# danieleschmidt/grid-fed-rl-gym

Measured on NVIDIA B200. Metric: env-steps/sec, higher is better.
Workload: dtype f64

## Files before the change

### grid-fed-rl-gym_b200/csrc/gfr_device.cuh

```cuda
#pragma once
#include <math.h>
#include <stdint.h>

#if defined(__CUDACC__)
#define GFR_HD __host__ __device__ __forceinline__
#else
#define GFR_HD inline
#endif

namespace gfr {

enum { SOLVER_SWEEP = 0, SOLVER_NEWTON = 1, SOLVER_SWEEP_TIES = 2 };
enum { BUS_SLACK = 0, BUS_PV = 1, BUS_PQ = 2 };
enum { GEN_SOLAR = 0, GEN_WIND = 1 };
enum { F_E = 0, F_F = 1, F_SCRATCH = 2 };
enum { S_JR = 2, S_P = 4 };
enum { SCRATCH_FIELDS_SWEEP = 2 };
enum { FL_PQ = 1, FL_FROM_IS_PARENT = 2, FL_FIXED_VM = 4, FL_THETA = 8,
       FL_SLACK_PATH = 16,
       FL_C_REG = 32,
       FL_P_REG = 64,
       FL_VALID = 128,
       FL_POOL_SHIFT = 8, FL_POOL_MASK = 0xFFF,
       FL_XSLOT_SHIFT = 20,
       REC_LIST_MASK = 0xFFFFF, REC_KIDX_SHIFT = 20 };
enum { R_TIME = 0, R_FREQ, R_WIND, R_TEMP, R_CLOUD, R_TOTAL_LOSSES, R_EPISODE_REWARD, R_SEED,
       R_DRAWS, R_COUNTS, R_BAT };

struct alignas(16) D2 { double x, y; };
struct alignas(16) I4 { int x, y, z, w; };
GFR_HD int pool_slot_of(int w) { return (w >> FL_POOL_SHIFT) & FL_POOL_MASK; }
GFR_HD int rec_bus(const I4& t) { return (int)((unsigned)t.x & 0xFFFFu); }
GFR_HD int rec_parent(const I4& t) { return (int)((unsigned)t.x >> 16); }
GFR_HD int rec_list(const I4& t) { return t.y & REC_LIST_MASK; }
GFR_HD int rec_kids_x_slot(const I4& t) { return (int)((unsigned)t.y >> REC_KIDX_SHIFT); }
GFR_HD int x_slot_of(int z) { return (int)((unsigned)z >> FL_XSLOT_SHIFT); }
GFR_HD int rec_pool_kids(const I4& t) { return (int)((unsigned)t.w & 0xFFFFu); }
GFR_HD int rec_all_kids(const I4& t) { return (int)((unsigned)t.w >> 16); }

struct Layout {
  int n, nl, L, G, Bt, A, D, m, n_src, R, img_bytes, n_noise, n_pool, k_slack;
  int nrows, P;
  int n_tie;
  int o_tie_ends, o_tie_ptr, o_tie_inc, o_tie_y, o_tie_z, o_tie_rating, o_tie_zinv;
  int o_sched, o_rank, o_rankp, o_branch_of_line, o_inj_ptr, o_inj_idx, o_gen_type;
  int o_gb, o_rating, o_vm_set;
  int o_child_ent, o_child_slot, o_gbd, o_f0;
  int o_kids;
  int o_topo, o_child_idx, o_rx;
  int o_rowrec, sw_rows;
  int o_load_base, o_gen_cap, o_gen_p0, o_gen_p1, o_gen_p2, o_bat_cap, o_bat_rating, o_bat_eff, o_profile;
  double s_base, inv_s_base, load_p_sum;
};

struct EnvCfg {
  double dt, v_min, v_max, f_min, f_max, penalty, load_noise, tol, accel;
  int episode_length, stochastic_loads, weather_variation, max_it;
};

struct SolveStat {
  double max_mismatch;
  int iterations;
  int converged;
};

GFR_HD uint64_t scratch_policy() {
#if defined(__CUDA_ARCH__) && !defined(GFR_NO_L2_POLICY)
  uint64_t pol;
  asm volatile("createpolicy.fractional.L2::evict_last.b64 %0, 1.0;" : "=l"(pol));
  return pol;
#else
  return 0;
#endif
}
GFR_HD D2 ld_scratch(const D2* p, uint64_t pol) {
#if defined(__CUDA_ARCH__) && !defined(GFR_NO_L2_POLICY)
  D2 r;
  asm volatile("ld.global.L1::no_allocate.L2::cache_hint.v2.f64 {%0, %1}, [%2], %3;" : "=d"(r.x), "=d"(r.y) : "l"(p), "l"(pol) : "memory");
  return r;
#elif defined(__CUDA_ARCH__)
  D2 r;
  asm volatile("ld.global.L1::no_allocate.v2.f64 {%0, %1}, [%2];" : "=d"(r.x), "=d"(r.y) : "l"(p) : "memory");
  return r;
#else
  (void)pol;
  return *p;
#endif
}
GFR_HD void st_scratch(D2* p, const D2 v, uint64_t pol) {
#if defined(__CUDA_ARCH__) && !defined(GFR_NO_L2_POLICY)
  asm volatile("st.global.L2::cache_hint.v2.f64 [%0], {%1, %2}, %3;" ::"l"(p), "d"(v.x), "d"(v.y), "l"(pol) : "memory");
// ... 353 lines not shown
template <class G, int LANES>
GFR_HD void flat_start_t(const G& g, const Lanes<LANES>&, const Layout& lay, const int* simg,
                         const double* dimg) {
  const I4* sched = reinterpret_cast<const I4*>(simg + lay.o_sched);
  if (wide_group<LANES>()) {
    for (int p0 = g.lane; p0 < lay.P; p0 += 4 * LANES) {
      I4 t[4]; double vs[4];
#pragma unroll
      for (int u = 0; u < 4; ++u) {
        const int p = p0 + u * LANES;
        t[u].x = t[u].y = t[u].z = t[u].w = 0; vs[u] = 1.0;
        if (p < lay.P) { t[u] = sched[p]; vs[u] = dimg[lay.o_vm_set + p]; }
      }
#pragma unroll
      for (int u = 0; u < 4; ++u) {
        if (!(t[u].z & FL_VALID)) continue;
        D2 v;
        v.x = (t[u].z & FL_FIXED_VM) ? vs[u] : 1.0;
        v.y = 0.0;
        g.ef(rec_bus(t[u])) = v;
      }
    }
  } else
  for (int p = g.lane; p < lay.P; p += LANES) {
    const I4 t = sched[p];
    if (!(t.z & FL_VALID)) continue;
    D2 v;
    v.x = (t.z & FL_FIXED_VM) ? dimg[lay.o_vm_set + p] : 1.0;
    v.y = 0.0;
    g.ef(rec_bus(t)) = v;
  }
  g.sync();
}
template <class G>
GFR_HD void flat_start(const G& g, const Layout& lay, const int* simg, const double* dimg) {
  flat_start_t(g, g, lay, simg, dimg);
}

#ifdef GFR_EMU_STATS
static long long gfr_emu_stats[4];
#endif
struct BranchT { double ga, al, gl, ll; };
GFR_HD BranchT branch_terms(const D2 vk, const D2 vp, const D2 y) {
  const double a = fma(vk.x, vp.x, vk.y * vp.y), s = fma(vk.y, vp.x, -vk.x * vp.y);
  BranchT t;
  t.ga = fma(-y.x, a, -y.y * s); t.al = fma(-y.x, s, y.y * a);
  t.gl = fma(-y.x, a, y.y * s);  t.ll = fma(y.x, s, y.y * a);
  return t;
}

GFR_HD unsigned shr16_pair(unsigned lo, unsigned hi) { return (lo >> 16) | (hi << 16); }
#define GFR_POOL_GATHER(t_, kq_, ...)                                                                              \
  do {                                                                                                             \
    const int npk_ = rec_pool_kids(t_);                                                                            \
    if (wide_group<LANES>() && npk_ <= 8) {                                                                       \
      unsigned w0_ = (unsigned)(kq_).x, w1_ = (unsigned)(kq_).y, w2_ = (unsigned)(kq_).z, w3_ = (unsigned)(kq_).w; \
      _Pragma("unroll 1")                                                                                          \
      for (int j_ = 0; j_ < npk_; ++j_) {                                                                          \
        const int slot = (int)(w0_ & 0xffffu);                                                                     \
        w0_ = shr16_pair(w0_, w1_); w1_ = shr16_pair(w1_, w2_); w2_ = shr16_pair(w2_, w3_); w3_ >>= 16;            \
        __VA_ARGS__                                                                                                \
      }                                                                                                            \
    } else {                                                                                                       \
      const int q1_ = rec_list(t_) + rec_all_kids(t_);                                                             \
      _Pragma("unroll 1")                                                                                          \
      for (int q_ = q1_ - npk_; q_ < q1_; ++q_) {                                                                  \
        const int slot = child_slot[q_];                                                                           \
        __VA_ARGS__                                                                                                \
      }                                                                                                            \
    }                                                                                                              \
  } while (0)

#define GFR_ROW_PIPE_DECL                                                                                          \
  I4 t_next, kq_next; D2 y_next, yd_next, vk_next, vp_next;                                                        \
  t_next.x = t_next.y = t_next.z = t_next.w = 0;                                                                   \
  kq_next = t_next;                                                                                                \
  y_next.x = y_next.y = yd_next.x = yd_next.y = vk_next.x = vk_next.y = vp_next.x = vp_next.y = 0.0
#define GFR_ROW_PIPE_LOAD(pos_)                                                                                    \
  do {                                                                                                             \
    t_next = sched[(pos_)]; y_next = gb[(pos_)]; yd_next = gbd[(pos_)];                                            \
    if (wide_group<LANES>()) kq_next = kids[(pos_)];                                                              \
    if (GFR_PIPE_EF) { vk_next = g.ef(rec_bus(t_next)); vp_next = g.ef(rec_parent(t_next)); }                      \
  } while (0)
#define GFR_ROW_PIPE_FIRST(pos_)                                                                                   \
  do { if (pipe_rows<LANES>()) GFR_ROW_PIPE_LOAD(pos_); } while (0)
#define GFR_ROW_PIPE_TAKE(p_, more_, next_)                                                                        \
  I4 t, kq; D2 yb, yd, vk, vp;                                                                                     \
  kq.x = kq.y = kq.z = kq.w = 0;                                                                                   \
  if (pipe_rows<LANES>()) {                                                                                        \
    t = t_next; yb = y_next; yd = yd_next; kq = kq_next;                                                           \
    if (GFR_PIPE_EF) { vk = vk_next; vp = vp_next; } else { vk = g.ef(rec_bus(t)); vp = g.ef(rec_parent(t)); }     \
    if (more_) GFR_ROW_PIPE_LOAD(next_);                                                                           \
  } else {                                                                                                         \
    t = sched[(p_)]; yb = gb[(p_)]; yd = gbd[(p_)]; vk = g.ef(rec_bus(t)); vp = g.ef(rec_parent(t));               \
    if (wide_group<LANES>()) kq = kids[(p_)];                                                                     \
  }

template <int LANES>
GFR_HD double newton_mismatch(const NGrp<LANES>& g, const Layout& lay, const int* simg, const double* dimg) {
  const int nrows = lay.nrows, np = lay.n_pool;
  const I4* sched = reinterpret_cast<const I4*>(simg + lay.o_sched);
  const int* child_slot = simg + lay.o_child_slot;
  const D2* gb = reinterpret_cast<const D2*>(dimg + lay.o_gb);
  const D2* gbd = reinterpret_cast<const D2*>(dimg + lay.o_gbd);
  const I4* kids = reinterpret_cast<const I4*>(simg + (wide_group<LANES>() ? lay.o_kids : 0));
  double mm = 0.0;
  D2 hf; hf.x = hf.y = 0.0;
  double ps_next = g.pspec((nrows - 1) * LANES + g.lane);
  GFR_ROW_PIPE_DECL;
  GFR_ROW_PIPE_FIRST((nrows - 1) * LANES + g.lane);
  for (int row = nrows - 1; row >= 0; --row) {
    const int p = row * LANES + g.lane;
    GFR_ROW_PIPE_TAKE(p, row > 0, p - LANES);
    const double ps = ps_next;
    if (row > 0) ps_next = g.pspec(p - LANES);
    if (t.z & FL_VALID) {
      const double v2 = fma(vk.x, vk.x, vk.y * vk.y);
      const BranchT bt = branch_terms(vk, vp, yb);
      if (!(t.z & FL_C_REG)) { hf.x = hf.y = 0.0; }
      GFR_POOL_GATHER(t, kq, {
        const D2 fl = g.poolp[3 * np + slot];
        hf.x += fl.x; hf.y += fl.y;
      });
      const double P = fma(yd.x, v2, bt.ga) + hf.x, Q = fma(-yd.y, v2, bt.al) + hf.y;
      double aP = fabs(ps - P), aQ = fabs(Q);
      if ((t.z & (FL_PQ | FL_THETA)) != (FL_PQ | FL_THETA)) {
        if (!(t.z & FL_THETA)) aP = 0.0;
        if (!(t.z & FL_PQ)) aQ = 0.0;
      }
      const double loc = (aQ > aP || aQ != aQ) ? aQ : aP;
      mm = (loc > mm || loc != loc) ? loc : mm;
      hf.x = bt.gl; hf.y = bt.ll;
      if (!(t.z & FL_P_REG)) g.poolp[3 * np + pool_slot_of(t.z)] = hf;
    }
    g.sync();
  }
  return g.gmax_nan(mm);
}

template <int LANES>
GFR_HD void newton_back_update(const NGrp<LANES>& g, const Layout& lay, const int* simg, const D2* f0,
                               double accel) {
  const int nrows = lay.nrows, P = lay.P;
  const I4* sched = reinterpret_cast<const I4*>(simg + lay.o_sched);
  D2 a0, a1, av, b0, b1, bv;
  a0.x = a0.y = a1.x = a1.y = b0.x = b0.y = b1.x = b1.y = bv.x = bv.y = 0.0;
#define GFR_LOAD_MV(row_, m0_, m1_, v_)                                    \
  do {                                                                     \
    const int ps_ = (row_) * LANES + g.lane;                               \
    if (!f0) { m0_ = ld_scratch(g.mg + ps_, g.pol); m1_ = ld_scratch(g.mg + P + ps_, g.pol); } \
    v_ = ld_scratch(g.mg + 2 * P + ps_, g.pol);                                   \
  } while (0)
  D2 hx; hx.x = hx.y = 0.0;
#define GFR_BU_ROW(row_, m0_, m1_, v_)                                     \
  do {                                                                     \
    const int p = (row_) * LANES + g.lane;                                 \
    I4 t;                                                                  \
    D2 e_now;                                                              \
    if (pipe_rows<LANES>()) {                                              \
      t = t_next; e_now = e_next;                                          \
      if ((row_) + 1 < nrows) { t_next = sched[p + LANES]; if (GFR_PIPE_EF) e_next = g.efp[rec_bus(t_next)]; } \
      if (!GFR_PIPE_EF) e_now = g.efp[rec_bus(t)];                         \
    } else { t = sched[p]; e_now = g.efp[rec_bus(t)]; }                    \
    D2 m0 = m0_, m1 = m1_, v = v_;                                         \
    if (f0) {                                                              \
      if (LANES > 32) {                                                    \
        m0 = f0m0_next; m1 = f0m1_next;                                    \
        if ((row_) + 1 < nrows) { f0m0_next = f0[2 * P + p + LANES]; f0m1_next = f0[3 * P + p + LANES]; } \
      } else { m0 = f0[2 * P + p]; m1 = f0[3 * P + p]; }                   \
    }                                                                      \
    if ((row_) + 2 < nrows) GFR_LOAD_MV((row_) + 2, m0_, m1_, v_);         \
    if (t.z & FL_VALID) {                                                  \
      D2 x = hx;                                                           \
      if (!(t.z & FL_P_REG)) x = g.poolp[x_slot_of(t.z)];                  \
      v.x = fma(-m0.x, x.x, fma(-m0.y, x.y, v.x));                         \
      v.y = fma(-m1.x, x.x, fma(-m1.y, x.y, v.y));                         \
      if (rec_pool_kids(t)) g.poolp[rec_kids_x_slot(t)] = v;               \
      hx = v;                                                              \
      double sn, cs;                                                       \
      sincos_small(accel * v.x, &sn, &cs);                                 \
      const double sc = fma(accel, v.y, 1.0);                              \
      D2* const ep = g.efp + rec_bus(t);                                   \
      const D2 e = e_now;                                                  \
      D2 w;                                                                \
      w.x = sc * fma(e.x, cs, -e.y * sn);                                  \
      w.y = sc * fma(e.x, sn, e.y * cs);                                   \
      *ep = w;                                                             \
    }                                                                      \
    g.sync();                                                              \
  } while (0)
  GFR_LOAD_MV(0, a0, a1, av);
  if (nrows > 1) GFR_LOAD_MV(1, b0, b1, bv);
  I4 t_next;
  t_next.x = t_next.y = t_next.z = t_next.w = 0;
  D2 f0m0_next, f0m1_next;
  f0m0_next.x = f0m0_next.y = f0m1_next.x = f0m1_next.y = 0.0;
  D2 e_next; e_next.x = e_next.y = 0.0;
  if (pipe_rows<LANES>()) { t_next = sched[g.lane]; if (GFR_PIPE_EF) e_next = g.efp[rec_bus(t_next)]; }
  if (LANES > 32 && f0) { f0m0_next = f0[2 * P + g.lane]; f0m1_next = f0[3 * P + g.lane]; }
  for (int row = 0; row < nrows; row += 2) {
    GFR_BU_ROW(row, a0, a1, av);
    if (row + 1 < nrows) GFR_BU_ROW(row + 1, b0, b1, bv);
  }
#undef GFR_BU_ROW
#undef GFR_LOAD_MV
}

template <int LANES>
GFR_HD void newton_solve(const NGrp<LANES>& g, const Layout& lay, const int* simg,
                         const double* dimg, double tol, int max_it, double accel,
                         SolveStat* out) {
  const int nrows = lay.nrows, np = lay.n_pool, P = lay.P;
  const I4* sched = reinterpret_cast<const I4*>(simg + lay.o_sched);
  const int* child_slot = simg + lay.o_child_slot;
  const D2* gb = reinterpret_cast<const D2*>(dimg + lay.o_gb);
  const D2* gbd = reinterpret_cast<const D2*>(dimg + lay.o_gbd);
  const D2* f0 = lay.o_f0 >= 0 ? reinterpret_cast<const D2*>(dimg + lay.o_f0) : nullptr;
  const I4* kids = reinterpret_cast<const I4*>(simg + (wide_group<LANES>() ? lay.o_kids : 0));

  out->converged = 0;
  out->iterations = max_it;
  out->max_mismatch = INFINITY;
  double mm_prev = INFINITY, rate = 1.0;

  for (int it = 0; it < max_it; ++it) {
    double mm;
    if (it == 0 && f0 != nullptr) {
      mm = 0.0;
      for (int p = g.lane; p < P; p += LANES) {
        const int fl = sched[p].z;
// ... 4 lines not shown
        const double loc = (aQ > aP || aQ != aQ) ? aQ : aP;
        if (fl & FL_VALID) mm = (loc > mm || loc != loc) ? loc : mm;
      }
      mm = g.gmax_nan(mm);
      out->max_mismatch = mm;
      if (mm < tol) {
        out->converged = 1;
        out->iterations = it + 1;
        break;
      }
      D2 hc; hc.x = hc.y = 0.0;
      double ps_next = g.pspec((nrows - 1) * LANES + g.lane);
      I4 t_next, kq_next; D2 pc_next, i0_next, i1_next, lp_next;
      t_next.x = t_next.y = t_next.z = t_next.w = 0;
      kq_next = t_next;
      pc_next.x = pc_next.y = i0_next.x = i0_next.y = i1_next.x = i1_next.y = lp_next.x = lp_next.y = 0.0;
      if (pipe_rows<LANES>()) {
        const int p0 = (nrows - 1) * LANES + g.lane;
        t_next = sched[p0]; pc_next = f0[5 * P + p0]; i0_next = f0[p0]; i1_next = f0[P + p0]; lp_next = f0[4 * P + p0];
        if (wide_group<LANES>()) kq_next = kids[p0];
      }
      for (int row = nrows - 1; row >= 0; --row) {
        const int p = row * LANES + g.lane;
        I4 t, kq; D2 pc, i0, i1, lp;
        kq.x = kq.y = kq.z = kq.w = 0;
        if (pipe_rows<LANES>()) {
          t = t_next; pc = pc_next; i0 = i0_next; i1 = i1_next; lp = lp_next; kq = kq_next;
          if (row > 0) {
            if (wide_group<LANES>()) kq_next = kids[p - LANES];
            t_next = sched[p - LANES]; pc_next = f0[5 * P + p - LANES];
            i0_next = f0[p - LANES]; i1_next = f0[P + p - LANES]; lp_next = f0[4 * P + p - LANES];
          }
        } else {
          t = sched[p]; pc = f0[5 * P + p]; i0 = f0[p]; i1 = f0[P + p]; lp = f0[4 * P + p];
          if (wide_group<LANES>()) kq = kids[p];
        }
        const double ps = ps_next;
        if (row > 0) ps_next = g.pspec(p - LANES);
        if (t.z & FL_VALID) {
          if (!(t.z & FL_C_REG)) { hc.x = hc.y = 0.0; }
          GFR_POOL_GATHER(t, kq, {
            const D2 cc = g.poolp[2 * np + slot];
            hc.x += cc.x; hc.y += cc.y;
          });
          const D2 sc = hc;
          double r0 = ps - pc.x - sc.x, r1 = 0.0 - pc.y - sc.y;
          if (!(t.z & FL_THETA)) r0 = 0.0;
          if (!(t.z & FL_PQ)) r1 = 0.0;
          D2 v;
          v.x = fma(i0.x, r0, i0.y * r1);
          v.y = fma(i1.x, r0, i1.y * r1);
          hc.x = fma(lp.x, v.x, lp.y * v.y);
          hc.y = fma(-lp.y, v.x, lp.x * v.y);
          st_scratch(g.mg + 2 * P + p, v, g.pol);
          if (!(t.z & FL_P_REG)) g.poolp[2 * np + pool_slot_of(t.z)] = hc;
        }
        g.sync();
      }
      newton_back_update(g, lay, simg, f0, accel);
    } else {
      if (rate * mm_prev * mm_prev < 0.25 * tol) {
#ifdef GFR_EMU_STATS
        ++gfr_emu_stats[0];
#endif
        mm = newton_mismatch(g, lay, simg, dimg);
        if (mm < tol) {
          out->max_mismatch = mm;
          out->converged = 1;
          out->iterations = it + 1;
          break;
        }
      }
      mm = 0.0;
      int singular = 0;
      D2 h0, h1, hc, hf;
      h0.x = h0.y = h1.x = h1.y = hc.x = hc.y = hf.x = hf.y = 0.0;
      double ps_next = g.pspec((nrows - 1) * LANES + g.lane);
      GFR_ROW_PIPE_DECL;
      GFR_ROW_PIPE_FIRST((nrows - 1) * LANES + g.lane);
      for (int row = nrows - 1; row >= 0; --row) {
        const int p = row * LANES + g.lane;
        GFR_ROW_PIPE_TAKE(p, row > 0, p - LANES);
        const double ps = ps_next;
        if (row > 0) ps_next = g.pspec(p - LANES);
        if (t.z & FL_VALID) {
          const double v2 = fma(vk.x, vk.x, vk.y * vk.y);
          const BranchT bt = branch_terms(vk, vp, yb);
          if (!(t.z & FL_C_REG)) { h0.x = h0.y = h1.x = h1.y = hc.x = hc.y = hf.x = hf.y = 0.0; }
          GFR_POOL_GATHER(t, kq, {
            const D2* e = g.poolp + slot;
            const D2 c0 = e[0], c1 = e[np], cc = e[2 * np], fl = e[3 * np];
            h0.x += c0.x; h0.y += c0.y; h1.x += c1.x; h1.y += c1.y; hc.x += cc.x; hc.y += cc.y;
            hf.x += fl.x; hf.y += fl.y;
          });
          const D2 s0 = h0, s1 = h1, sc = hc, sf = hf;
          const double Pk = fma(yd.x, v2, bt.ga) + sf.x, Q = fma(-yd.y, v2, bt.al) + sf.y;
          D2 d0, d1, r;
          r.x = ps - Pk;
          r.y = 0.0 - Q;
          double aP = fabs(r.x), aQ = fabs(Q);
          r.x -= sc.x; r.y -= sc.y;
          d0.x = fma(-yd.y, v2, -Q) - s0.x;
          d0.y = fma(yd.x, v2, Pk) - s0.y;
          d1.x = fma(-yd.x, v2, Pk) - s1.x;
          d1.y = fma(-yd.y, v2, Q) - s1.y;
          double u00 = bt.al, u01 = bt.ga, u10 = -bt.ga, u11 = bt.al;
          if ((t.z & (FL_PQ | FL_THETA)) != (FL_PQ | FL_THETA)) {
            if (!(t.z & FL_THETA)) { aP = 0.0; d0.x = 1.0; d0.y = 0.0; r.x = 0.0; u00 = 0.0; u01 = 0.0; }
            if (!(t.z & FL_PQ)) { aQ = 0.0; d1.x = 0.0; d1.y = 1.0; r.y = 0.0; u10 = 0.0; u11 = 0.0; }
          }
          const double loc = (aQ > aP || aQ != aQ) ? aQ : aP;
          mm = (loc > mm || loc != loc) ? loc : mm;
          const double det = fma(d0.x, d1.y, -d0.y * d1.x);
          if (det == 0.0) singular = 1;
          const double inv = rcp_fast(det);
          const double i00 = d1.y * inv, i01 = -d0.y * inv, i10 = -d1.x * inv, i11 = d0.x * inv;
          D2 m0, m1, v;
          m0.x = fma(i00, u00, i01 * u10);
          m0.y = fma(i00, u01, i01 * u11);
          m1.x = fma(i10, u00, i11 * u10);
          m1.y = fma(i10, u01, i11 * u11);
          v.x = fma(i00, r.x, i01 * r.y);
          v.y = fma(i10, r.x, i11 * r.y);
          st_scratch(g.mg + p, m0, g.pol);
          st_scratch(g.mg + P + p, m1, g.pol);
          st_scratch(g.mg + 2 * P + p, v, g.pol);
          h0.x = fma(bt.ll, m0.x, bt.gl * m1.x);
          h0.y = fma(bt.ll, m0.y, bt.gl * m1.y);
          h1.x = fma(-bt.gl, m0.x, bt.ll * m1.x);
          h1.y = fma(-bt.gl, m0.y, bt.ll * m1.y);
          hc.x = fma(bt.ll, v.x, bt.gl * v.y);
          hc.y = fma(-bt.gl, v.x, bt.ll * v.y);
          hf.x = bt.gl; hf.y = bt.ll;
          if (!(t.z & FL_P_REG)) {
            D2* const own = g.poolp + pool_slot_of(t.z);
            own[0] = h0; own[np] = h1; own[2 * np] = hc; own[3 * np] = hf;
          }
        }
        g.sync();
      }
      mm = g.gmax_nan(mm);
#ifdef GFR_EMU_STATS
      ++gfr_emu_stats[1];
      if (mm < tol) ++gfr_emu_stats[2];
#endif
      out->max_mismatch = mm;
      if (mm < tol) {
        out->converged = 1;
        out->iterations = it + 1;
        break;
      }
      if (g.gor(singular)) {
        out->iterations = it + 1;
        break;
      }
      newton_back_update(g, lay, simg, (const D2*)nullptr, accel);
    }
    {
      const double q = mm / (mm_prev * mm_prev);
      rate = (q > 1e-3 && q < 1e3) ? q : ((q >= 1e3) ? 1e3 : 1.0);
      mm_prev = mm;
    }
  }
#if defined(__CUDA_ARCH__) && GFR_SCRATCH_DISCARD
  {
    char* const base = reinterpret_cast<char*>(g.mg);
#if GFR_SCRATCH_DISCARD == 2
    const size_t bytes = ((size_t)P * 48) & ~(size_t)127;
#else
    const size_t bytes = newton_scratch_doubles(P) * 8;
#endif
    for (size_t off = (size_t)g.lane * 128; off < bytes; off += (size_t)LANES * 128)
      asm volatile("discard.global.L2 [%0], 128;" ::"l"(base + off) : "memory");
  }
#endif
}

template <int LANES, bool TIES>
GFR_HD void sweep_solve(const SGrp<LANES>& g, const Layout& lay, const int* simg,
                        const double* dimg, double tol, int max_it, SolveStat* out) {
  const int n = lay.n, nrows = lay.sw_rows, ks = lay.k_slack, nt = TIES ? lay.n_tie : 0;
  const I4* topo = reinterpret_cast<const I4*>(simg + lay.o_topo);
  const I4* rowrec = reinterpret_cast<const I4*>(simg + (LANES > 1 ? lay.o_rowrec : 0));
  const int* child_idx = simg + lay.o_child_idx;
  const int* tie_ptr = simg + lay.o_tie_ptr;
  const int* tie_inc = simg + lay.o_tie_inc;
// ... 704 lines not shown
```

### grid-fed-rl-gym_b200/csrc/gfr_image.hpp

```cpp
#pragma once
#include <algorithm>
#include <cstring>
#include <string>
#include <vector>

#include "../../include/gfr_b200.h"
#include "gfr_device.cuh"

namespace gfr {

struct ImageBuilder {
  std::vector<int32_t> ints;
  std::vector<double> dbls;
  int add_i(const int32_t* p, int count) {
    while (ints.size() % 4) ints.push_back(0);
    int off = (int)ints.size();
    if (count > 0) ints.insert(ints.end(), p, p + count);
    return off;
  }
  int add_d(const double* p, int count) {
    if (dbls.size() % 2) dbls.push_back(0.0);
    int off = (int)dbls.size();
    if (count > 0) dbls.insert(dbls.end(), p, p + count);
    return off;
// ... 197 lines not shown
  for (int l = 0; l < L; ++l) lp = lp + d->load_p[l];
  lay.load_p_sum = lp;

  Schedule sch;
  std::vector<int> pos(n);
  if (newton) {
    sch = make_schedule(d, lanes);
    for (int k = 0; k < n; ++k) pos[k] = sch.row[k] * lanes + sch.lane[k];
    lay.nrows = sch.nrows;
    lay.P = sch.nrows * lanes;
    if (lay.P > 65535) return "more than 65535 schedule positions";
  } else {
    for (int k = 0; k < n; ++k) pos[k] = k;
    lay.nrows = nl;
    lay.P = n;
  }
  const int P = lay.P;
  std::vector<int> bus_at(P, -1);
  for (int k = 0; k < n; ++k) bus_at[pos[k]] = k;

  std::vector<int32_t> flags(n), rank(n), rankp(n), bol(lay.m > 0 ? lay.m : 0);
  for (int i = 0; i < nt; ++i) bol[d->tie_line[i]] = -1 - i;
  for (int k = 0; k < n; ++k) {
    int fl = FL_VALID;
    if (d->bus_type[k] == GFR_BUS_PQ) fl |= FL_PQ;
    else fl |= FL_FIXED_VM;
    if (d->bus_type[k] != GFR_BUS_SLACK) fl |= FL_THETA;
    if (d->bus_type[k] == GFR_BUS_PV) f->has_pv = true;
    if (d->from_is_parent[k]) fl |= FL_FROM_IS_PARENT;
    flags[k] = fl;
    rank[d->order[k]] = k;
    rankp[d->order[k]] = pos[k];
    if (k > 0) bol[d->line_of[k]] = pos[k];
  }
  {
    int ks = 0;
    for (int k = 0; k < n; ++k) if (d->bus_type[k] == GFR_BUS_SLACK) ks = k;
    lay.k_slack = ks;
    for (int k = ks; k > 0; k = d->parent[k]) flags[k] |= FL_SLACK_PATH;
  }
  std::vector<int> heir(n, -1);
  if (newton) {
    for (int k = 1; k < n; ++k) {
      const int p = d->parent[k];
      if (sch.row[k] == sch.row[p] + 1 && sch.lane[k] == sch.lane[p] && heir[p] < 0) {
        heir[p] = k;
        flags[p] |= FL_C_REG;
        flags[k] |= FL_P_REG;
        ++f->n_reg_edges;
      }
    }
    flags[0] |= FL_P_REG;
  }
  std::vector<int32_t> pool_slot(n, 0);
  lay.n_pool = 1;
  if (newton) {
    std::vector<std::vector<int>> by_row(sch.nrows);
    for (int k = 0; k < n; ++k) by_row[sch.row[k]].push_back(k);
    std::vector<int> free_slots;
    int np = 0;
    for (int r = sch.nrows - 1; r >= 0; --r) {
      std::vector<int> released;
      for (int k : by_row[r])
        for (int q = d->child_ptr[k]; q < d->child_ptr[k + 1]; ++q) {
          const int c = d->child_idx[q];
          if (c != heir[k]) released.push_back(pool_slot[c]);
        }
      for (int k : by_row[r]) {
        if (flags[k] & FL_P_REG) continue;
        if (!free_slots.empty()) {
          auto it = std::min_element(free_slots.begin(), free_slots.end());
          pool_slot[k] = *it;
          free_slots.erase(it);
        } else {
          pool_slot[k] = np++;
        }
      }
      free_slots.insert(free_slots.end(), released.begin(), released.end());
    }
    lay.n_pool = std::max(np, 1);
    if (d->n_pool > lay.n_pool) lay.n_pool = d->n_pool;
    if (lay.n_pool > FL_POOL_MASK) return "more than 4095 pool slots";
  }
  std::vector<int32_t> kids_x_slot(n, 0), x_slot(n, 0);
  if (newton) {
    for (int k = 0; k < n; ++k) {
      int best = -1;
      for (int q = d->child_ptr[k]; q < d->child_ptr[k + 1]; ++q) {
        const int c = d->child_idx[q];
        if (c != heir[k] && (best < 0 || sch.row[c] > sch.row[best])) best = c;
      }
      if (best >= 0) {
        kids_x_slot[k] = pool_slot[best];
        for (int q = d->child_ptr[k]; q < d->child_ptr[k + 1]; ++q)
          if (d->child_idx[q] != heir[k]) x_slot[d->child_idx[q]] = pool_slot[best];
      }
    }
  }

  ImageBuilder ib;
  std::vector<int32_t> sched(4 * (size_t)P, 0), child_ent, child_slot;
  std::vector<int32_t> topo(4 * (size_t)n);
  for (int p = 0; p < P; ++p) {
    const int k = bus_at[p];
    if (k < 0) continue;
    const int kp = k > 0 ? d->parent[k] : 0;
    const int begin = (int)child_ent.size();
    int n_pool_kids = 0, n_all = 0;
    if (newton) {
      for (int pass = 0; pass < 2; ++pass)
        for (int q = d->child_ptr[k]; q < d->child_ptr[k + 1]; ++q) {
          const int c = d->child_idx[q];
          if ((c == heir[k]) != (pass == 0)) continue;
          child_ent.push_back((int32_t)((uint32_t)c | ((uint32_t)pos[c] << 16)));
          child_slot.push_back(pool_slot[c]);
          ++n_all;
          if (pass == 1) ++n_pool_kids;
        }
      if (n_all > 65535) return "more than 65535 children on one bus";
    }
    sched[4 * p + 0] = (int32_t)((uint32_t)k | ((uint32_t)kp << 16));
    if (begin > REC_LIST_MASK) return "child lists too long";
    sched[4 * p + 1] = (int32_t)((uint32_t)begin | ((uint32_t)kids_x_slot[k] << REC_KIDX_SHIFT));
    sched[4 * p + 2] = (int32_t)((uint32_t)flags[k] | ((uint32_t)pool_slot[k] << FL_POOL_SHIFT) | ((uint32_t)x_slot[k] << FL_XSLOT_SHIFT));
    sched[4 * p + 3] = (int32_t)((uint32_t)n_pool_kids | ((uint32_t)n_all << 16));
  }
  for (int k = 0; k < n; ++k) {
    topo[4 * k + 0] = k > 0 ? d->parent[k] : 0;
    topo[4 * k + 1] = d->child_ptr[k];
    topo[4 * k + 2] = d->child_ptr[k + 1];
    topo[4 * k + 3] = flags[k];
  }
  lay.o_sched = ib.add_i(sched.data(), 4 * P);
  std::vector<int32_t> inj_ptr(P + 1, 0), inj_idx(lay.n_src);
  {
    std::vector<int> cnt(P, 0);
    for (int l = 0; l < L; ++l) cnt[pos[d->load_bus[l]]]++;
    for (int g = 0; g < G; ++g) cnt[pos[d->gen_bus[g]]]++;
    for (int b = 0; b < Bt; ++b) cnt[pos[d->bat_bus[b]]]++;
    for (int p = 0; p < P; ++p) inj_ptr[p + 1] = inj_ptr[p] + cnt[p];
    std::vector<int> fill(inj_ptr.begin(), inj_ptr.end() - 1);
    for (int l = 0; l < L; ++l) inj_idx[fill[pos[d->load_bus[l]]]++] = l;
    for (int g = 0; g < G; ++g) inj_idx[fill[pos[d->gen_bus[g]]]++] = L + g;
    for (int b = 0; b < Bt; ++b) inj_idx[fill[pos[d->bat_bus[b]]]++] = L + G + b;
  }
  lay.o_rank = ib.add_i(rank.data(), n);
  lay.o_rankp = newton ? ib.add_i(rankp.data(), n) : lay.o_rank;
  lay.o_branch_of_line = ib.add_i(bol.data(), lay.m);
  lay.o_inj_ptr = ib.add_i(inj_ptr.data(), P + 1);
  lay.o_inj_idx = ib.add_i(inj_idx.data(), lay.n_src);
  lay.o_gen_type = ib.add_i(d->gen_type, G);
  lay.o_child_ent = lay.o_child_slot = lay.o_topo = lay.o_child_idx = -1;
  lay.o_kids = -1;
  lay.o_rowrec = -1; lay.sw_rows = 0;
  if (newton) {
    lay.o_child_slot = ib.add_i(child_slot.data(), (int)child_slot.size());
    if (lanes >= GFR_WIDE_GROUP_MIN_LANES) {
      std::vector<int32_t> kids(4 * (size_t)P, 0);
      for (int p = 0; p < P; ++p) {
        const uint32_t begin = (uint32_t)sched[4 * p + 1] & (uint32_t)REC_LIST_MASK;
        const uint32_t npk = (uint32_t)sched[4 * p + 3] & 0xffffu, nall = (uint32_t)sched[4 * p + 3] >> 16;
        for (uint32_t j = 0; j < npk && j < 8; ++j) {
          const uint32_t slot = (uint32_t)child_slot[begin + nall - npk + j];
          kids[4 * p + (j >> 1)] = (int32_t)((uint32_t)kids[4 * p + (j >> 1)] | (slot << (16 * (j & 1))));
        }
      }
      lay.o_kids = ib.add_i(kids.data(), 4 * P);
    }
  } else {
    lay.o_topo = ib.add_i(topo.data(), 4 * n);
    lay.o_child_idx = ib.add_i(d->child_idx, n - 1);
    if (lanes > 1) {
      const Schedule sw = make_schedule(d, lanes);
      std::vector<int32_t> rowrec(4 * (size_t)sw.nrows * lanes, 0);
      for (int k = 0; k < n; ++k) {
        int32_t* r = &rowrec[4 * ((size_t)sw.row[k] * lanes + sw.lane[k])];
        r[0] = (int32_t)((uint32_t)k | ((uint32_t)(k > 0 ? d->parent[k] : 0) << 16));
        r[1] = d->child_ptr[k];
        r[2] = d->child_ptr[k + 1];
        r[3] = flags[k];
      }
      lay.sw_rows = sw.nrows;
      lay.o_rowrec = ib.add_i(rowrec.data(), (int)rowrec.size());
    }
  }
  lay.o_tie_ends = lay.o_tie_ptr = lay.o_tie_inc = lay.o_tie_y = lay.o_tie_z = lay.o_tie_rating = lay.o_tie_zinv = -1;
  if (nt) {
    std::vector<int32_t> ends(2 * (size_t)nt), tptr(n + 1, 0), tinc(2 * (size_t)nt);
    std::vector<int> cnt(n, 0);
    for (int i = 0; i < nt; ++i) { ends[2 * i] = d->tie_from[i]; ends[2 * i + 1] = d->tie_to[i]; cnt[d->tie_from[i]]++; cnt[d->tie_to[i]]++; }
    for (int k = 0; k < n; ++k) tptr[k + 1] = tptr[k] + cnt[k];
    std::vector<int> fill(tptr.begin(), tptr.end() - 1);
    for (int i = 0; i < nt; ++i) { tinc[fill[d->tie_from[i]]++] = i << 1; tinc[fill[d->tie_to[i]]++] = (i << 1) | 1; }
    lay.o_tie_ends = ib.add_i(ends.data(), 2 * nt);
    lay.o_tie_ptr = ib.add_i(tptr.data(), n + 1);
    lay.o_tie_inc = ib.add_i(tinc.data(), 2 * nt);
  }
  const int n_int_padded = ((int)ib.ints.size() + 3) / 4 * 4;
  const int dbase = n_int_padded / 2;
  std::vector<double> gb(2 * (size_t)P, 0.0), gbd(2 * (size_t)P, 0.0), rx(2 * (size_t)P, 0.0), rating(P, 0.0), vm_set(P, 1.0);
  for (int k = 0; k < n; ++k) {
    const int p = pos[k];
    gb[2 * p] = k > 0 ? d->g[k] : 0.0; gb[2 * p + 1] = k > 0 ? d->b[k] : 0.0;
    gbd[2 * p] = d->gdiag[k]; gbd[2 * p + 1] = d->bdiag[k];
    rx[2 * p] = d->r[k]; rx[2 * p + 1] = d->x[k];
    rating[p] = d->rating[k];
    vm_set[p] = d->vm_set[k];
  }
  lay.o_gb = dbase + ib.add_d(gb.data(), 2 * P);
  lay.o_gbd = lay.o_rx = lay.o_f0 = -1;
  if (newton) lay.o_gbd = dbase + ib.add_d(gbd.data(), 2 * P);
  else lay.o_rx = dbase + ib.add_d(rx.data(), 2 * P);
  if (newton) {
    std::vector<double> f0(12 * (size_t)P, 0.0), C(4 * (size_t)n, 0.0);
    bool ok = flat_start_factors;
    for (int k = n - 1; k >= 0 && ok; --k) {
// ... 83 lines not shown
```

### grid-fed-rl-gym_b200/topology.py

```python

from __future__ import annotations

from dataclasses import dataclass, field
from typing import Any, Dict, List, Optional, Sequence, Tuple

import os
import numpy as np

IEEE13_ZERO_LENGTH_PU: Dict[str, Tuple[float, float]] = {
    "line_633_634": (0.0, 0.06),
    "line_671_692": (1e-4, 1e-4),
}

OPEN_Z = 1e-12


class TopologyError(ValueError):
    """The feeder cannot be compiled for the radial solvers."""


class RepairedFeeder:

    def __init__(self, source, lines: List[Any], dropped: List[Any], added: List[Any]) -> None:
        self.name = getattr(source, "name", type(source).__name__)
# ... 193 lines not shown
        raise TopologyError("feeder is not connected (run repair_topology first)")
    pending = [0] * n
    for v in bfs[1:]:
        pending[parent_ref[v][0]] += 1
    ready = [v for v in bfs if pending[v] == 0]
    steps = []
    while ready:
        ready.sort(key=lambda v: (-depth[v], v))
        take = ready if width is None else ready[:width]
        rest = [] if width is None else ready[width:]
        steps.append(take)
        for v in take:
            u = parent_ref[v][0]
            if u >= 0:
                pending[u] -= 1
                if pending[u] == 0:
                    rest.append(u)
        ready = rest
    steps.reverse()
    assert steps[0] == [root]
    level = {}
    for l, members in enumerate(steps):
        for v in members:
            level[v] = l
    if not alap:
        bfs_moves = []
    else:
        bfs_moves = bfs[1:]
    room = [None if width is None else width - len(members) for members in steps]
    for v in bfs_moves:
        target = level[parent_ref[v][0]] + 1
        cur = level[v]
        while target < cur:
            if room[target] is None or room[target] > 0:
                if room[target] is not None:
                    room[target] -= 1
                    room[cur] += 1
                level[v] = target
                break
            target += 1
    steps = [[] for _ in steps]
    for v in bfs:
        steps[level[v]].append(v)
    assert all(steps) and steps[0] == [root]
    order, level_of, pos = [], {}, {-1: -1}
    for l, members in enumerate(steps):
        for v in sorted(members, key=lambda v: (pos[parent_ref[v][0]], v)):
            level_of[v] = l
            pos[v] = len(order)
            order.append(v)
    return order, parent_ref, level_of


def _schedule_paths(n: int, root: int, adj, width: int):
    parent_ref = {root: (-1, -1)}
    depth = {root: 0}
    bfs = [root]
    for u in bfs:
        for v, k in adj[u]:
            if v not in parent_ref:
                parent_ref[v] = (u, k)
                depth[v] = depth[u] + 1
                bfs.append(v)
    if len(bfs) != n:
        raise TopologyError("feeder is not connected (run repair_topology first)")
    pending = [0] * n
    for v in bfs[1:]:
        pending[parent_ref[v][0]] += 1
    ready = set(v for v in bfs if pending[v] == 0)
    last = [None] * width
    steps = []
    while ready:
        cont = {}
        for lane in range(width):
            b = last[lane]
            if b is not None:
                u = parent_ref[b][0]
                if u >= 0 and u in ready and u not in cont:
                    cont[u] = lane
        take = sorted(ready, key=lambda v: (0 if v in cont else 1, -depth[v], v))[:width]
        assign = {v: cont[v] for v in take if v in cont}
        free = [lane for lane in range(width) if lane not in assign.values()]
        for v in take:
            if v not in assign:
                assign[v] = free.pop(0)
        last = [None] * width
        for v, lane in assign.items():
            last[lane] = v
            ready.discard(v)
        for v in assign:
            u = parent_ref[v][0]
            if u >= 0:
                pending[u] -= 1
                if pending[u] == 0:
                    ready.add(u)
        steps.append(assign)
    steps.reverse()
    assert list(steps[0]) == [root]
    row_of = {v: l for l, assign in enumerate(steps) for v in assign}
    has_kids = set(parent_ref[v][0] for v in bfs[1:])
    for v in sorted((v for v in bfs[1:] if v not in has_kids), key=lambda v: -(row_of[v] - row_of[parent_ref[v][0]])):
        u = parent_ref[v][0]
        cur = row_of[v]
        if cur == row_of[u] + 1 and steps[cur][v] == steps[row_of[u]].get(u):
            continue
        for r in range(row_of[u] + 1, cur):
            if len(steps[r]) < width:
                lane = min(set(range(width)) - set(steps[r].values()))
                del steps[cur][v]
                steps[r][v] = lane
                row_of[v] = r
                break
    order, level_of, lane_of = [], {}, {}
    for l, assign in enumerate(steps):
        for v in sorted(assign, key=lambda v: assign[v]):
            level_of[v] = l
            lane_of[v] = assign[v]
            order.append(v)
    return order, parent_ref, level_of, lane_of


def tree_center(n: int, adj, fallback: int) -> int:
    def far(s):
        dist = {s: 0}
        q = [s]
        for u in q:
            for v, _ in adj[u]:
                if v not in dist:
                    dist[v] = dist[u] + 1
                    q.append(v)
        t = max(dist, key=lambda v: (dist[v], -v))
        return t, dist
    if n == 1:
        return fallback
    a, _ = far(fallback)
    b, da = far(a)
    path = [b]
    while path[-1] != a:
        u = path[-1]
        path.append(next(v for v, _ in adj[u] if da[v] == da[u] - 1))
    return path[len(path) // 2]


def compile_feeder(feeder, renewable_sources: Optional[Sequence[str]] = None,
                   with_components: bool = True, root: str = "slack",
                   width: Optional[int] = None, paths: bool = False) -> FeederSoA:
    buses, lines = list(feeder.buses), list(feeder.lines)
    n, m = len(buses), len(lines)
    if n < 1:
        raise TopologyError("feeder has no buses")
    if m < n - 1:
        raise TopologyError(f"a connected feeder needs at least n-1 lines, this one has {n} buses and {m} lines "
                            "(run repair_topology first)")
    index = {b.id: i for i, b in enumerate(buses)}
    if len(index) != n:
        raise TopologyError("duplicate bus ids")
    slack = _slack_index(buses)

    adj: List[List[Tuple[int, int]]] = [[] for _ in range(n)]
    ydiag = np.zeros(n, dtype=complex)
    ys: List[complex] = []
    uf = list(range(n))
    ties: List[int] = []

    def _find(a: int) -> int:
# ... 191 lines not shown
```

Baseline: 98.43 million.

## Chain sibling subtree contributions through pool slots so parents gather fewer tails

For wide lane groups, non-heir children of a bus are arranged into chains where each child absorbs an earlier sibling's pooled contribution, so the parent gathers only chain tails instead of every child. The pool-slot lifetimes and the kids_x slot allocation are recomputed from actual reader rows, and the Python leaf scheduler places leaves on rows that spread siblings apart so chains can form. The aim is to cut the serial gather work and pool memory traffic at high-fanout buses. In exchange, each absorbing row does an extra dependent pool load, and the host-side slot allocation becomes more complex.

New measurement: 101.8 million (median of 6 runs). 3.4% higher.

```diff
diff --git a/grid-fed-rl-gym_b200/csrc/gfr_device.cuh b/grid-fed-rl-gym_b200/csrc/gfr_device.cuh
--- a/grid-fed-rl-gym_b200/csrc/gfr_device.cuh
+++ b/grid-fed-rl-gym_b200/csrc/gfr_device.cuh
@@ -33,10 +33,12 @@
 GFR_HD int rec_bus(const I4& t) { return (int)((unsigned)t.x & 0xFFFFu); }
 GFR_HD int rec_parent(const I4& t) { return (int)((unsigned)t.x >> 16); }
 GFR_HD int rec_list(const I4& t) { return t.y & REC_LIST_MASK; }
-GFR_HD int rec_kids_x_slot(const I4& t) { return (int)((unsigned)t.y >> REC_KIDX_SHIFT); }
+GFR_HD int rec_kids_x_slot(const I4& t) { return (int)((unsigned)t.y >> REC_KIDX_SHIFT) - 1; }
 GFR_HD int x_slot_of(int z) { return (int)((unsigned)z >> FL_XSLOT_SHIFT); }
-GFR_HD int rec_pool_kids(const I4& t) { return (int)((unsigned)t.w & 0xFFFFu); }
-GFR_HD int rec_all_kids(const I4& t) { return (int)((unsigned)t.w >> 16); }
+GFR_HD int rec_tails(const I4& t) { return (int)((unsigned)t.w & 0xFFFFu); }
+GFR_HD int rec_absorb(const I4& t) { return (int)((unsigned)t.w >> 16) - 1; }
+enum { CHAIN_MIN_LANES = 8 };
+template <int LANES> GFR_HD constexpr bool sibling_chains() { return LANES >= CHAIN_MIN_LANES; }
 
 struct Layout {
   int n, nl, L, G, Bt, A, D, m, n_src, R, img_bytes, n_noise, n_pool, k_slack;
@@ -496,7 +498,7 @@
 GFR_HD unsigned shr16_pair(unsigned lo, unsigned hi) { return (lo >> 16) | (hi << 16); }
 #define GFR_POOL_GATHER(t_, kq_, ...)                                                                              \
   do {                                                                                                             \
-    const int npk_ = rec_pool_kids(t_);                                                                            \
+    const int npk_ = rec_tails(t_);                                                                                \
     if (wide_group<LANES>() && npk_ <= 8) {                                                                       \
       unsigned w0_ = (unsigned)(kq_).x, w1_ = (unsigned)(kq_).y, w2_ = (unsigned)(kq_).z, w3_ = (unsigned)(kq_).w; \
       _Pragma("unroll 1")                                                                                          \
@@ -506,9 +508,9 @@
         __VA_ARGS__                                                                                                \
       }                                                                                                            \
     } else {                                                                                                       \
-      const int q1_ = rec_list(t_) + rec_all_kids(t_);                                                             \
+      const int q0_ = rec_list(t_);                                                                                \
       _Pragma("unroll 1")                                                                                          \
-      for (int q_ = q1_ - npk_; q_ < q1_; ++q_) {                                                                  \
+      for (int q_ = q0_; q_ < q0_ + npk_; ++q_) {                                                                  \
         const int slot = child_slot[q_];                                                                           \
         __VA_ARGS__                                                                                                \
       }                                                                                                            \
@@ -575,6 +577,10 @@
       const double loc = (aQ > aP || aQ != aQ) ? aQ : aP;
       mm = (loc > mm || loc != loc) ? loc : mm;
       hf.x = bt.gl; hf.y = bt.ll;
+      if (sibling_chains<LANES>() && rec_absorb(t) >= 0) {
+        const D2 fl = g.poolp[3 * np + rec_absorb(t)];
+        hf.x += fl.x; hf.y += fl.y;
+      }
       if (!(t.z & FL_P_REG)) g.poolp[3 * np + pool_slot_of(t.z)] = hf;
     }
     g.sync();
@@ -619,7 +625,7 @@
       if (!(t.z & FL_P_REG)) x = g.poolp[x_slot_of(t.z)];                  \
       v.x = fma(-m0.x, x.x, fma(-m0.y, x.y, v.x));                         \
       v.y = fma(-m1.x, x.x, fma(-m1.y, x.y, v.y));                         \
-      if (rec_pool_kids(t)) g.poolp[rec_kids_x_slot(t)] = v;               \
+      if (rec_kids_x_slot(t) >= 0) g.poolp[rec_kids_x_slot(t)] = v;        \
       hx = v;                                                              \
       double sn, cs;                                                       \
       sincos_small(accel * v.x, &sn, &cs);                                 \
@@ -730,6 +736,10 @@
           v.y = fma(i1.x, r0, i1.y * r1);
           hc.x = fma(lp.x, v.x, lp.y * v.y);
           hc.y = fma(-lp.y, v.x, lp.x * v.y);
+          if (sibling_chains<LANES>() && rec_absorb(t) >= 0) {
+            const D2 cc = g.poolp[2 * np + rec_absorb(t)];
+            hc.x += cc.x; hc.y += cc.y;
+          }
           st_scratch(g.mg + 2 * P + p, v, g.pol);
           if (!(t.z & FL_P_REG)) g.poolp[2 * np + pool_slot_of(t.z)] = hc;
         }
@@ -800,9 +810,6 @@
           m1.y = fma(i10, u01, i11 * u11);
           v.x = fma(i00, r.x, i01 * r.y);
           v.y = fma(i10, r.x, i11 * r.y);
-          st_scratch(g.mg + p, m0, g.pol);
-          st_scratch(g.mg + P + p, m1, g.pol);
-          st_scratch(g.mg + 2 * P + p, v, g.pol);
           h0.x = fma(bt.ll, m0.x, bt.gl * m1.x);
           h0.y = fma(bt.ll, m0.y, bt.gl * m1.y);
           h1.x = fma(-bt.gl, m0.x, bt.ll * m1.x);
@@ -810,6 +817,15 @@
           hc.x = fma(bt.ll, v.x, bt.gl * v.y);
           hc.y = fma(-bt.gl, v.x, bt.ll * v.y);
           hf.x = bt.gl; hf.y = bt.ll;
+          if (sibling_chains<LANES>() && rec_absorb(t) >= 0) {
+            const D2* e = g.poolp + rec_absorb(t);
+            const D2 c0 = e[0], c1 = e[np], cc = e[2 * np], fl = e[3 * np];
+            h0.x += c0.x; h0.y += c0.y; h1.x += c1.x; h1.y += c1.y; hc.x += cc.x; hc.y += cc.y;
+            hf.x += fl.x; hf.y += fl.y;
+          }
+          st_scratch(g.mg + p, m0, g.pol);
+          st_scratch(g.mg + P + p, m1, g.pol);
+          st_scratch(g.mg + 2 * P + p, v, g.pol);
           if (!(t.z & FL_P_REG)) {
             D2* const own = g.poolp + pool_slot_of(t.z);
             own[0] = h0; own[np] = h1; own[2 * np] = hc; own[3 * np] = hf;
diff --git a/grid-fed-rl-gym_b200/csrc/gfr_image.hpp b/grid-fed-rl-gym_b200/csrc/gfr_image.hpp
--- a/grid-fed-rl-gym_b200/csrc/gfr_image.hpp
+++ b/grid-fed-rl-gym_b200/csrc/gfr_image.hpp
@@ -273,20 +273,58 @@
     }
     flags[0] |= FL_P_REG;
   }
+  std::vector<int> absorb(n, -1), reader_row(n, -1);
+  std::vector<std::vector<int>> tails(n);
+  if (newton) {
+    std::vector<int> kids;
+    for (int k = 0; k < n; ++k) {
+      kids.clear();
+      for (int q = d->child_ptr[k]; q < d->child_ptr[k + 1]; ++q)
+        if (d->child_idx[q] != heir[k]) kids.push_back(d->child_idx[q]);
+      if (lanes < CHAIN_MIN_LANES) {
+        tails[k] = kids;
+        for (int c : kids) reader_row[c] = sch.row[k];
+        continue;
+      }
+      std::stable_sort(kids.begin(), kids.end(), [&](int a, int b) { return sch.row[a] > sch.row[b]; });
+      std::vector<int>& open = tails[k];
+      for (size_t i = 0; i < kids.size();) {
+        const int r = sch.row[kids[i]];
+        size_t j = i;
+        size_t avail = open.size();
+        std::vector<int> started;
+        for (; j < kids.size() && sch.row[kids[j]] == r; ++j) {
+          const int c = kids[j];
+          if (avail > 0) {
+            absorb[c] = open.front();
+            reader_row[open.front()] = r;
+            open.erase(open.begin());
+            --avail;
+          }
+          started.push_back(c);
+        }
+        open.insert(open.end(), started.begin(), started.end());
+        i = j;
+      }
+      if (heir[k] >= 0 && !open.empty() && sch.row[open.front()] > sch.row[heir[k]]) {
+        absorb[heir[k]] = open.front();
+        reader_row[open.front()] = sch.row[heir[k]];
+        open.erase(open.begin());
+      }
+      for (int c : open) reader_row[c] = sch.row[k];
+    }
+  }
   std::vector<int32_t> pool_slot(n, 0);
   lay.n_pool = 1;
   if (newton) {
-    std::vector<std::vector<int>> by_row(sch.nrows);
-    for (int k = 0; k < n; ++k) by_row[sch.row[k]].push_back(k);
+    std::vector<std::vector<int>> by_row(sch.nrows), read_in(sch.nrows);
+    for (int k = 0; k < n; ++k) {
+      by_row[sch.row[k]].push_back(k);
+      if (reader_row[k] >= 0) read_in[reader_row[k]].push_back(k);
+    }
     std::vector<int> free_slots;
     int np = 0;
     for (int r = sch.nrows - 1; r >= 0; --r) {
-      std::vector<int> released;
-      for (int k : by_row[r])
-        for (int q = d->child_ptr[k]; q < d->child_ptr[k + 1]; ++q) {
-          const int c = d->child_idx[q];
-          if (c != heir[k]) released.push_back(pool_slot[c]);
-        }
       for (int k : by_row[r]) {
         if (flags[k] & FL_P_REG) continue;
         if (!free_slots.empty()) {
@@ -297,54 +335,56 @@
           pool_slot[k] = np++;
         }
       }
-      free_slots.insert(free_slots.end(), released.begin(), released.end());
+      for (int k : read_in[r]) free_slots.push_back(pool_slot[k]);
     }
     lay.n_pool = std::max(np, 1);
+  }
+  std::vector<int32_t> kids_x_slot(n, -1), x_slot(n, 0);
+  if (newton) {
+    std::vector<int> last_read(n, -1);
+    for (int k = 1; k < n; ++k)
+      if (k != heir[d->parent[k]]) last_read[d->parent[k]] = std::max(last_read[d->parent[k]], sch.row[k]);
+    std::vector<std::vector<int>> by_row(sch.nrows), freed_after(sch.nrows);
+    for (int k = 0; k < n; ++k)
+      if (last_read[k] >= 0) { by_row[sch.row[k]].push_back(k); freed_after[last_read[k]].push_back(k); }
+    std::vector<int> free_slots;
+    int np = 0;
+    for (int r = 0; r < sch.nrows; ++r) {
+      if (r > 0)
+        for (int k : freed_after[r - 1]) free_slots.push_back(kids_x_slot[k]);
+      for (int k : by_row[r]) {
+        if (!free_slots.empty()) {
+          auto it = std::min_element(free_slots.begin(), free_slots.end());
+          kids_x_slot[k] = *it;
+          free_slots.erase(it);
+        } else {
+          kids_x_slot[k] = np++;
+        }
+      }
+    }
+    for (int k = 1; k < n; ++k)
+      if (k != heir[d->parent[k]]) x_slot[k] = kids_x_slot[d->parent[k]];
+    lay.n_pool = std::max(lay.n_pool, np);
     if (d->n_pool > lay.n_pool) lay.n_pool = d->n_pool;
     if (lay.n_pool > FL_POOL_MASK) return "more than 4095 pool slots";
   }
-  std::vector<int32_t> kids_x_slot(n, 0), x_slot(n, 0);
-  if (newton) {
-    for (int k = 0; k < n; ++k) {
-      int best = -1;
-      for (int q = d->child_ptr[k]; q < d->child_ptr[k + 1]; ++q) {
-        const int c = d->child_idx[q];
-        if (c != heir[k] && (best < 0 || sch.row[c] > sch.row[best])) best = c;
-      }
-      if (best >= 0) {
-        kids_x_slot[k] = pool_slot[best];
-        for (int q = d->child_ptr[k]; q < d->child_ptr[k + 1]; ++q)
-          if (d->child_idx[q] != heir[k]) x_slot[d->child_idx[q]] = pool_slot[best];
-      }
-    }
-  }
 
   ImageBuilder ib;
-  std::vector<int32_t> sched(4 * (size_t)P, 0), child_ent, child_slot;
+  std::vector<int32_t> sched(4 * (size_t)P, 0), child_slot;
   std::vector<int32_t> topo(4 * (size_t)n);
   for (int p = 0; p < P; ++p) {
     const int k = bus_at[p];
     if (k < 0) continue;
     const int kp = k > 0 ? d->parent[k] : 0;
-    const int begin = (int)child_ent.size();
-    int n_pool_kids = 0, n_all = 0;
-    if (newton) {
-      for (int pass = 0; pass < 2; ++pass)
-        for (int q = d->child_ptr[k]; q < d->child_ptr[k + 1]; ++q) {
-          const int c = d->child_idx[q];
-          if ((c == heir[k]) != (pass == 0)) continue;
-          child_ent.push_back((int32_t)((uint32_t)c | ((uint32_t)pos[c] << 16)));
-          child_slot.push_back(pool_slot[c]);
-          ++n_all;
-          if (pass == 1) ++n_pool_kids;
-        }
-      if (n_all > 65535) return "more than 65535 children on one bus";
-    }
+    const int begin = (int)child_slot.size();
+    for (int c : tails[k]) child_slot.push_back(pool_slot[c]);
+    const int n_tails = (int)tails[k].size();
+    if (n_tails > 65535) return "more than 65535 chain tails on one bus";
     sched[4 * p + 0] = (int32_t)((uint32_t)k | ((uint32_t)kp << 16));
     if (begin > REC_LIST_MASK) return "child lists too long";
-    sched[4 * p + 1] = (int32_t)((uint32_t)begin | ((uint32_t)kids_x_slot[k] << REC_KIDX_SHIFT));
+    sched[4 * p + 1] = (int32_t)((uint32_t)begin | ((uint32_t)(kids_x_slot[k] + 1) << REC_KIDX_SHIFT));
     sched[4 * p + 2] = (int32_t)((uint32_t)flags[k] | ((uint32_t)pool_slot[k] << FL_POOL_SHIFT) | ((uint32_t)x_slot[k] << FL_XSLOT_SHIFT));
-    sched[4 * p + 3] = (int32_t)((uint32_t)n_pool_kids | ((uint32_t)n_all << 16));
+    sched[4 * p + 3] = (int32_t)((uint32_t)n_tails | ((uint32_t)(absorb[k] >= 0 ? pool_slot[absorb[k]] + 1 : 0) << 16));
   }
   for (int k = 0; k < n; ++k) {
     topo[4 * k + 0] = k > 0 ? d->parent[k] : 0;
@@ -380,9 +420,9 @@
       std::vector<int32_t> kids(4 * (size_t)P, 0);
       for (int p = 0; p < P; ++p) {
         const uint32_t begin = (uint32_t)sched[4 * p + 1] & (uint32_t)REC_LIST_MASK;
-        const uint32_t npk = (uint32_t)sched[4 * p + 3] & 0xffffu, nall = (uint32_t)sched[4 * p + 3] >> 16;
-        for (uint32_t j = 0; j < npk && j < 8; ++j) {
-          const uint32_t slot = (uint32_t)child_slot[begin + nall - npk + j];
+        const uint32_t nt = (uint32_t)sched[4 * p + 3] & 0xffffu;
+        for (uint32_t j = 0; j < nt && j < 8; ++j) {
+          const uint32_t slot = (uint32_t)child_slot[begin + j];
           kids[4 * p + (j >> 1)] = (int32_t)((uint32_t)kids[4 * p + (j >> 1)] | (slot << (16 * (j & 1))));
         }
       }
diff --git a/grid-fed-rl-gym_b200/topology.py b/grid-fed-rl-gym_b200/topology.py
--- a/grid-fed-rl-gym_b200/topology.py
+++ b/grid-fed-rl-gym_b200/topology.py
@@ -269,6 +269,9 @@
     return order, parent_ref, level_of
 
 
+CHAIN_MIN_LANES = 8
+
+
 def _schedule_paths(n: int, root: int, adj, width: int):
     parent_ref = {root: (-1, -1)}
     depth = {root: 0}
@@ -316,18 +319,30 @@
     assert list(steps[0]) == [root]
     row_of = {v: l for l, assign in enumerate(steps) for v in assign}
     has_kids = set(parent_ref[v][0] for v in bfs[1:])
+    kids_of = {}
+    for v in bfs[1:]:
+        kids_of.setdefault(parent_ref[v][0], []).append(v)
+
+    def is_heir(v):
+        u = parent_ref[v][0]
+        return row_of[v] == row_of[u] + 1 and steps[row_of[v]][v] == steps[row_of[u]].get(u)
+
     for v in sorted((v for v in bfs[1:] if v not in has_kids), key=lambda v: -(row_of[v] - row_of[parent_ref[v][0]])):
         u = parent_ref[v][0]
         cur = row_of[v]
-        if cur == row_of[u] + 1 and steps[cur][v] == steps[row_of[u]].get(u):
+        if is_heir(v):
             continue
-        for r in range(row_of[u] + 1, cur):
-            if len(steps[r]) < width:
-                lane = min(set(range(width)) - set(steps[r].values()))
-                del steps[cur][v]
-                steps[r][v] = lane
-                row_of[v] = r
-                break
+        rows = [r for r in range(row_of[u] + 1, cur + 1) if r == cur or len(steps[r]) < width]
+        if width >= CHAIN_MIN_LANES:
+            sibs = [row_of[w] for w in kids_of[u] if w != v and not is_heir(w)]
+            r = min(rows, key=lambda r: (sibs.count(r), r))
+        else:
+            r = rows[0]
+        if r != cur:
+            lane = min(set(range(width)) - set(steps[r].values()))
+            del steps[cur][v]
+            steps[r][v] = lane
+            row_of[v] = r
     order, level_of, lane_of = [], {}, {}
     for l, assign in enumerate(steps):
         for v in sorted(assign, key=lambda v: assign[v]):
```
